# dropbox/divans

Measured on AMD Instinct MI355X. Metric: MB/s encode+decode per GPU, 64 KiB metablocks; bit-exact vs CPU, higher is better.
Workload: dtype u16/u64 integer

## Files before the change

### divans_amd/csrc/lit_bucket.hip

```cpp
#include "lit_bucket_dev.h"

namespace divans_hip {

__global__ __launch_bounds__(BK_SORT_THREADS) void bucket_sort_kernel(const BucketBatch b) {
    __shared__ __attribute__((aligned(16))) uint8_t staging[BK_PIECE];
    __shared__ __attribute__((aligned(16))) uint8_t piece_in[16 + BK_PIECE];
    __shared__ uint32_t hist[4][256];
    __shared__ uint32_t scan[256];
    const uint32_t s = blockIdx.x / b.pieces, piece = blockIdx.x % b.pieces;
    const uint32_t tid = threadIdx.x, w = tid >> 6, lane = tid & 63;
    const uint32_t len = b.in_sizes ? b.in_sizes[s] : b.stream_len;
    const uint8_t* in = b.in + (b.in_offsets ? b.in_offsets[s] : (uint64_t)s * b.stream_len);
    uint32_t* desc = b.desc + ((size_t)s * 256u + tid) * 8u + piece;
    const uint32_t base = piece * BK_PIECE;
    if (base >= len) { *desc = 0u; return; }
    const uint32_t n = len - base < BK_PIECE ? len - base : BK_PIECE;
    const size_t pl = b.slot;
    for (uint32_t i = tid; i < 1024u; i += BK_SORT_THREADS) (&hist[0][0])[i] = 0u;
    {
        const uint8_t* src = in + base;
        if ((((uintptr_t)src) & 15u) == 0u) {
            for (uint32_t i = tid * 16u; i < n; i += BK_SORT_THREADS * 16u) {
                if (i + 16u <= n) *(u32x4*)(piece_in + 16u + i) = *(const u32x4*)(src + i);
                else for (uint32_t k = i; k < n; ++k) piece_in[16u + k] = src[k];
            }
        } else {
            for (uint32_t i = tid; i < n; i += BK_SORT_THREADS) piece_in[16u + i] = src[i];
        }
        if (tid == 0u) piece_in[15] = base ? in[base - 1u] : 0u;
    }
    __syncthreads();
    const uint8_t* key_of = piece_in + 15;
    for (uint32_t bt = 0; bt < 32u; ++bt) {
        const uint32_t p = w * 2048u + bt * 64u + lane;
        if (p < n) atomicAdd(&hist[w][key_of[p]], 1u);
    }
    __syncthreads();
    const uint32_t c0 = hist[0][tid], c1 = hist[1][tid], c2 = hist[2][tid], c3 = hist[3][tid];
    const uint32_t tot = c0 + c1 + c2 + c3;
    scan[tid] = tot;
    __syncthreads();
    for (uint32_t d = 1; d < 256u; d <<= 1) {
        const uint32_t v = tid >= d ? scan[tid - d] : 0u;
        __syncthreads();
        scan[tid] += v;
        __syncthreads();
    }
    const uint32_t start = scan[tid] - tot;
    hist[0][tid] = start; hist[1][tid] = start + c0; hist[2][tid] = start + c0 + c1; hist[3][tid] = start + c0 + c1 + c2;
    *desc = start | (tot << 16);
    __syncthreads();
    uint16_t* inv = b.inv + (size_t)s * pl + base;
    for (uint32_t bt = 0; bt < 32u; ++bt) {
        const uint32_t p = w * 2048u + bt * 64u + lane;
        const bool valid = p < n;
        const uint32_t key = valid ? key_of[p] : 0u;
        const uint32_t byte = valid ? key_of[p + 1u] : 0u;
        unsigned long long same = __ballot(valid);
        for (uint32_t bit = 0; bit < 8u; ++bit) {
            const bool set = (key >> bit) & 1u;
            const unsigned long long bb = __ballot(set);
            same &= set ? bb : ~bb;
        }
        const uint32_t rank = lanes_below(same), cnt = (uint32_t)__popcll(same);
        if (valid) {
            const uint32_t off = hist[w][key];
            staging[off + rank] = (uint8_t)byte;
            inv[p] = (uint16_t)(off + rank);
            if (rank == cnt - 1u) hist[w][key] = off + cnt;
        }
    }
    __syncthreads();
    uint8_t* sorted = b.sorted + (size_t)s * pl + base;
    for (uint32_t i = tid * 16u; i < n; i += BK_SORT_THREADS * 16u) {
        if (i + 16u <= n) *(u32x4*)(sorted + i) = *(const u32x4*)(staging + i);
        else for (uint32_t k = i; k < n; ++k) sorted[k] = staging[k];
    }
}

__global__ __launch_bounds__(1024) void bucket_tasks_kernel(const BucketBatch b) {
    __shared__ uint32_t cnt[BK_CLASSES], basev[BK_CLASSES];
    const uint32_t t = blockIdx.x * 1024u + threadIdx.x;
    const uint32_t cap = b.n_streams * 256u;
    if (threadIdx.x < BK_CLASSES) cnt[threadIdx.x] = 0u;
    __syncthreads();
    uint32_t tot = 0;
    if (t < cap) {
        const u32x4* d = (const u32x4*)(b.desc + (size_t)t * 8u);
        const u32x4 d0 = d[0], d1 = d[1];
        tot = (d0.x >> 16) + (d0.y >> 16) + (d0.z >> 16) + (d0.w >> 16) + (d1.x >> 16) + (d1.y >> 16) + (d1.z >> 16) + (d1.w >> 16);
    }
    const int cls = bk_class_of(tot);
    uint32_t local = 0;
    for (int c = 0; c < (int)BK_CLASSES; ++c) {
        const unsigned long long m = __ballot(cls == c);
        if (m == 0ull) continue;
        const int leader = __ffsll((long long)m) - 1;
        uint32_t wbase = 0;
        if ((int)(threadIdx.x & 63u) == leader) wbase = atomicAdd(&cnt[c], (uint32_t)__popcll(m));
        wbase = (uint32_t)__builtin_amdgcn_readlane((int)wbase, leader);
        if (cls == c) local = wbase + lanes_below(m);
    }
    __syncthreads();
    if (threadIdx.x < BK_CLASSES) basev[threadIdx.x] = cnt[threadIdx.x] ? atomicAdd(&b.counters[threadIdx.x], cnt[threadIdx.x]) : 0u;
    __syncthreads();
    if (cls >= 0) b.tasks[(size_t)cls * cap + basev[cls] + local] = t;
}

__global__ __launch_bounds__(64) void bucket_chain_kernel(const BucketBatch b) {
    extern __shared__ __attribute__((aligned(16))) uint32_t lds32[];
    const uint32_t lane = threadIdx.x;
    uint32_t* my = lds32 + lane * BK_LANE_DWORDS;
    uint32_t* mydesc = my + BK_DESC_DW;
    uint32_t* tab = lds32 + BK_TAB_DW;
    const uint32_t inc = (uint32_t)b.inc; const int lim = b.lim;
    for (uint32_t i = lane; i < 128u; i += 64u) {
        const uint32_t sym = i >> 3, k = i & 7u;
        tab[i] = (2u * k >= sym ? inc : 0u) | (2u * k + 1u >= sym ? inc << 16 : 0u);
    }
    __syncthreads();
    const size_t pl = b.slot;
    const uint32_t cap = b.n_streams * 256u;
    BkTaskLists lists; lists.load(b.counters);
    const uint32_t total = lists.total();
    const u32x4 def0 = {4u | (8u << 16), 12u | (16u << 16), 20u | (24u << 16), 28u | (32u << 16)};
    const u32x4 def1 = {36u | (40u << 16), 44u | (48u << 16), 52u | (56u << 16), 60u | (64u << 16)};

    bool has_task = false, exhausted = false;
    uint32_t run_i = 0, nruns = 0, left = 0, idx = 0;
    u32x2* cur_sfs = b.sfs; const uint8_t* cur_sorted = b.sorted;
    uint32_t nt_stage = 0, nt_tid = 0;
    u32x4 nd0 = {0u, 0u, 0u, 0u}, nd1 = {0u, 0u, 0u, 0u};
    uint32_t win_cur = 0, win_end = 0, nxt_val = 0, nxt_w = 0;
    const uint32_t long_end = lists.ends[3];
    bool nxt_pending = false, drained = false;
    u32x2 e_next = {0u, 0u}; uint32_t m_next = 0;
    u32x2 pv0 = {0u, 0u}, pv1 = pv0, pv2 = pv0, pv3 = pv0, pv4 = pv0, pv5 = pv0, pv6 = pv0, pv7 = pv0;
    uint32_t m_prev = 0; u32x2* sfs_prev = b.sfs;

#define BK_OPAQUE(X) asm volatile("" : "+v"(X))
#define BK_BYTE(K, WORD, PV)                                                                            \
    if (((K - first) & 15u) < cnt) {                                                                    \
        const uint32_t byte_ = (WORD >> (8u * (K & 3u))) & 0xffu;                                       \
        const uint32_t hi = byte_ >> 4, lo = byte_ & 15u;                                               \
        uint32_t* rowl = my + 8u * (1u + hi);                                                           \
        BkRow H = bk_read(my, tab, hi), L = bk_read(rowl, tab, lo);                                     \
        const u32x2 v = {bk_pack(H, hi), bk_pack(L, lo)};                                               \
        H.w0 += H.a0; H.w1 += H.a1; L.w0 += L.a0; L.w1 += L.a1;           \
        if ((int)(H.w1.w >> 16) >= lim) bk_renorm(H);                                                   \
        if ((int)(L.w1.w >> 16) >= lim) bk_renorm(L);                                                   \
        *(u32x4*)my = H.w0; *(u32x4*)(my + 4) = H.w1; *(u32x4*)rowl = L.w0; *(u32x4*)(rowl + 4) = L.w1; \
        PV = v;                                                                                         \
    }

    for (;;) {
        u32x2 e = e_next; const uint32_t m = m_next;
        if (m_prev & BK_VALID) {
            u32x2* dst = sfs_prev + (m_prev & 0xffffu);
            const uint32_t pf = (m_prev >> 16) & 15u, pc = (m_prev >> 20) & 15u;
            if (pc == 8u) {
                const u32x4 q0 = {pv0.x, pv0.y, pv1.x, pv1.y}, q1 = {pv2.x, pv2.y, pv3.x, pv3.y};
                const u32x4 q2 = {pv4.x, pv4.y, pv5.x, pv5.y}, q3 = {pv6.x, pv6.y, pv7.x, pv7.y};
                bk_store_quad((u32x4*)dst, q0); bk_store_quad((u32x4*)(dst + 2), q1);
                bk_store_quad((u32x4*)(dst + 4), q2); bk_store_quad((u32x4*)(dst + 6), q3);
            } else {
                if (((0u - pf) & 15u) < pc) bk_store_pair(dst + 0, pv0);
                if (((1u - pf) & 15u) < pc) bk_store_pair(dst + 1, pv1);
                if (((2u - pf) & 15u) < pc) bk_store_pair(dst + 2, pv2);
                if (((3u - pf) & 15u) < pc) bk_store_pair(dst + 3, pv3);
                if (((4u - pf) & 15u) < pc) bk_store_pair(dst + 4, pv4);
                if (((5u - pf) & 15u) < pc) bk_store_pair(dst + 5, pv5);
                if (((6u - pf) & 15u) < pc) bk_store_pair(dst + 6, pv6);
                if (((7u - pf) & 15u) < pc) bk_store_pair(dst + 7, pv7);
            }
        }
        {
            const bool adv = has_task && left == 0u, more = run_i < nruns;
            const uint32_t d = mydesc[run_i & 7u];
            if (adv && more) { left = d >> 16; idx = d & 0xffffu; ++run_i; }
            if (adv && !more) has_task = false;
        }
        {
            const bool fetch_ = has_task && left != 0u;
            const uint32_t base = idx & ~7u, first_ = idx & 7u;
            const uint32_t cnt_ = left < 8u - first_ ? left : 8u - first_;
            const uint8_t* lp = fetch_ ? cur_sorted + base : b.sorted;
            e_next = *(const u32x2*)lp;
            m_next = fetch_ ? (base | (first_ << 16) | (cnt_ << 20) | BK_VALID) : 0u;
            idx += fetch_ ? cnt_ : 0u; left -= fetch_ ? cnt_ : 0u;
        }
        BK_OPAQUE(e);
        m_prev = m; sfs_prev = cur_sfs;
        if (m & BK_VALID) {
            const uint32_t first = (m >> 16) & 15u, cnt = (m >> 20) & 15u;
            BK_BYTE(0u, e.x, pv0) BK_BYTE(1u, e.x, pv1) BK_BYTE(2u, e.x, pv2) BK_BYTE(3u, e.x, pv3)
            BK_BYTE(4u, e.y, pv4) BK_BYTE(5u, e.y, pv5) BK_BYTE(6u, e.y, pv6) BK_BYTE(7u, e.y, pv7)
        }
        if (!has_task && !(m_next & BK_VALID) && nt_stage == 3u) {
            BK_OPAQUE(nd0); BK_OPAQUE(nd1);
            uint32_t n = 0;
            const uint32_t dsc[8] = {nd0.x, nd0.y, nd0.z, nd0.w, nd1.x, nd1.y, nd1.z, nd1.w};
#pragma unroll
            for (uint32_t j = 0; j < 8u; ++j) if (dsc[j] >> 16) { mydesc[n] = dsc[j] + j * BK_PIECE; ++n; }
            nruns = n; run_i = 0u;
            for (uint32_t r = 0; r < 17u; ++r) { *(u32x4*)(my + 8u * r) = def0; *(u32x4*)(my + 8u * r + 4u) = def1; }
            cur_sfs = b.sfs + (size_t)(nt_tid >> 8) * pl; cur_sorted = b.sorted + (size_t)(nt_tid >> 8) * pl;
            left = 0u; has_task = true; nt_stage = 0u;
        }
        const bool want = nt_stage == 0u && !exhausted;
        if (nt_stage == 2u) nt_stage = 3u;
        else if (nt_stage == 1u) {
            BK_OPAQUE(nt_tid);
            const u32x4* dp = (const u32x4*)(b.desc + (size_t)nt_tid * 8u);
            nd0 = dp[0]; nd1 = dp[1];
            nt_stage = 2u;
        }
        const unsigned long long wm = __ballot(want);
        if (wm) {
            if (win_cur == win_end && nxt_pending) {
                BK_OPAQUE(nxt_val);
                const uint32_t basev = (uint32_t)__builtin_amdgcn_readfirstlane((int)nxt_val);
                nxt_pending = false;
                if (basev >= total) { drained = true; win_cur = win_end = total; }
                else { win_cur = basev; win_end = basev + nxt_w < total ? basev + nxt_w : total; }
            }
            const uint32_t avail = win_end - win_cur, asked = (uint32_t)__popcll(wm);
            const uint32_t rank = lanes_below(wm);
            if (want) {
                if (rank < avail) {
                    const uint32_t t = win_cur + rank;
                    nt_tid = *lists.at(b.tasks, cap, t);
                    nt_stage = 1u;
                } else if (drained) exhausted = true;
            }
            win_cur += asked < avail ? asked : avail;
        }
        const uint32_t want_w = win_end < long_end ? 64u : BK_WINDOW;
        if (!nxt_pending && !drained && win_end - win_cur < want_w / 2u) {
            nxt_w = want_w;
            if (lane == 0u) nxt_val = atomicAdd(&b.counters[BK_CLAIM], want_w);
            nxt_pending = true;
        }
        const bool done = !has_task && !(m_next & BK_VALID) && !(m_prev & BK_VALID) && nt_stage == 0u && exhausted;
        if (__ballot(!done) == 0ull) break;
    }
#undef BK_BYTE
#undef BK_OPAQUE
}

__global__ __launch_bounds__(1024) void bucket_unsort_kernel(const BucketBatch b) {
    __shared__ u32x2 buf[BK_PIECE];
    const uint32_t s = blockIdx.x / b.pieces, piece = blockIdx.x % b.pieces;
    const uint32_t len = b.in_sizes ? b.in_sizes[s] : b.stream_len;
    const uint32_t base = piece * BK_PIECE;
    if (base >= len) return;
    const uint32_t n = len - base < BK_PIECE ? len - base : BK_PIECE;
    const size_t pl = b.slot;
    const u32x2* src = b.sfs + (size_t)s * pl + base;
    for (uint32_t i = threadIdx.x; i < n; i += 1024u) buf[i] = __builtin_nontemporal_load(src + i);
    __syncthreads();
    const uint16_t* inv = b.inv + (size_t)s * pl + base;
    u32x2* dst = (u32x2*)(b.sf + (size_t)s * b.sf_stride) + base;
    for (uint32_t i = threadIdx.x; i < n; i += 1024u) dst[i] = buf[inv[i]];
}

__global__ __launch_bounds__(1024) void bucket_unsort32_kernel(const BucketBatch b) {
    __shared__ uint32_t buf[BK_PIECE];
    const uint32_t s = blockIdx.x / b.pieces, piece = blockIdx.x % b.pieces;
    const uint32_t len = b.in_sizes ? b.in_sizes[s] : b.stream_len;
    const uint32_t base = piece * BK_PIECE;
    if (base >= len) return;
    const uint32_t n = len - base < BK_PIECE ? len - base : BK_PIECE;
    const size_t pl = b.slot;
    const uint32_t* src = (const uint32_t*)b.sfs + (size_t)s * pl + base;
    const uint32_t n2 = (n + 1u) & ~1u;
    for (uint32_t i = 2u * threadIdx.x; i < n2; i += 2048u) *(u32x2*)(buf + i) = __builtin_nontemporal_load((const u32x2*)(src + i));
    __syncthreads();
    const uint16_t* inv = b.inv + (size_t)s * pl + base;
    uint32_t* dst = b.sf + (size_t)s * b.sf_stride + base;
    for (uint32_t i = 2u * threadIdx.x; i < n2; i += 2048u) {
        const uint32_t iv = *(const uint32_t*)(inv + i);
        const u32x2 v = {buf[iv & 0xffffu], i + 1u < n ? buf[iv >> 16] : 0u};
        *(u32x2*)(dst + i) = v;
    }
}

uint32_t bucket_chain_lds_bytes() { return (64u * BK_LANE_DWORDS + 128u) * 4u; }

void launch_bucket_tasks(const BucketBatch& b, hipStream_t st) {
    hipLaunchKernelGGL(bucket_tasks_kernel, dim3((b.n_streams + 3u) / 4u), dim3(1024), 0, st, b);
}
void launch_bucket_unsort(const BucketBatch& b, hipStream_t st) {
    hipLaunchKernelGGL(bucket_unsort_kernel, dim3(b.n_streams * b.pieces), dim3(1024), 0, st, b);
}

void launch_bucket_unsort32(const BucketBatch& b, hipStream_t st) {
    hipLaunchKernelGGL(bucket_unsort32_kernel, dim3(b.n_streams * b.pieces), dim3(1024), 0, st, b);
}

hipError_t launch_bucket_model(const BucketBatch& b, uint32_t chain_blocks, hipStream_t st) {
    hipError_t e = hipMemsetAsync(b.counters, 0, 64, st);
    if (e != hipSuccess) return e;
    if (b.pieces < 8u) {
        e = hipMemsetAsync(b.desc, 0, (size_t)b.n_streams * 256u * 8u * sizeof(uint32_t), st);
        if (e != hipSuccess) return e;
    }
    hipLaunchKernelGGL(bucket_sort_kernel, dim3(b.n_streams * b.pieces), dim3(BK_SORT_THREADS), 0, st, b);
    hipLaunchKernelGGL(bucket_tasks_kernel, dim3((b.n_streams + 3u) / 4u), dim3(1024), 0, st, b);
    hipLaunchKernelGGL(bucket_chain_kernel, dim3(chain_blocks), dim3(64), bucket_chain_lds_bytes(), st, b);
    hipLaunchKernelGGL(bucket_unsort_kernel, dim3(b.n_streams * b.pieces), dim3(1024), 0, st, b);
    return hipGetLastError();
}

}
```

### divans_amd/csrc/lit_bucket_dev.h

```cpp
#ifndef DIVANS_LIT_BUCKET_DEV_H_
#define DIVANS_LIT_BUCKET_DEV_H_
#include "lit_device.h"

namespace divans_hip {

constexpr uint32_t BK_PIECE = 8192;
constexpr uint32_t BK_SORT_THREADS = 256;
constexpr uint32_t BK_LANE_DWORDS = 148;
constexpr uint32_t BK_DESC_DW = 136;
constexpr uint32_t BK_TAB_DW = 64 * BK_LANE_DWORDS;
constexpr uint32_t BK_VALID = 1u << 31;
constexpr uint32_t BK_WINDOW = 256;
constexpr uint32_t BK_CLASSES = 6;
constexpr uint32_t BK_CLAIM = 8;

__device__ __forceinline__ int bk_class_of(uint32_t tot) {
    return tot == 0u ? -1 : (tot >= 16384u ? 0 : (tot >= 8192u ? 1 : (tot >= 4096u ? 2 : (tot >= 2048u ? 3 : (tot >= 64u ? 4 : 5)))));
}
struct BkTaskLists {
    uint32_t ends[BK_CLASSES];
    __device__ __forceinline__ void load(const uint32_t* counters) {
        uint32_t acc = 0;
#pragma unroll
        for (uint32_t c = 0; c < BK_CLASSES; ++c) { acc += counters[c]; ends[c] = acc; }
    }
    __device__ __forceinline__ uint32_t total() const { return ends[BK_CLASSES - 1u]; }
    __device__ __forceinline__ const uint32_t* at(const uint32_t* tasks, uint32_t cap, uint32_t t) const {
        uint32_t cls = 0, base = 0;
#pragma unroll
        for (uint32_t c = 0; c + 1u < BK_CLASSES; ++c) if (t >= ends[c]) { cls = c + 1u; base = ends[c]; }
        return tasks + (size_t)cls * cap + (t - base);
    }
};

__device__ __forceinline__ uint32_t lanes_below(unsigned long long m) {
    return __builtin_amdgcn_mbcnt_hi((uint32_t)(m >> 32), __builtin_amdgcn_mbcnt_lo((uint32_t)m, 0u));
}

struct BkRow { u32x4 w0, w1, a0, a1; int chi, cprev; };

__device__ __forceinline__ BkRow bk_read(const uint32_t* row, const uint32_t* tab, uint32_t sym) {
    BkRow r;
    r.w0 = *(const u32x4*)row; r.w1 = *(const u32x4*)(row + 4);
    const uint16_t* r16 = (const uint16_t*)row;
    r.chi = r16[sym];
    r.cprev = r16[sym ? sym - 1u : 0u];
    r.a0 = *(const u32x4*)(tab + sym * 8u); r.a1 = *(const u32x4*)(tab + sym * 8u + 4u);
    return r;
}
__device__ __forceinline__ uint32_t bk_pack(const BkRow& r, uint32_t sym) {
    const int mx = (int)(r.w1.w >> 16);
    const int clo = sym ? r.cprev : 0;
    const float rcp = biased_rcp15(mx);
    const uint32_t dhi = scaled_div(r.chi, mx, rcp), dlo = scaled_div(clo, mx, rcp);
    return (dlo + 1u) | ((dhi - dlo - 1u) << 16);
}
__device__ __forceinline__ void bk_renorm(BkRow& r) {
    const u32x4 b0 = {1u | (2u << 16), 3u | (4u << 16), 5u | (6u << 16), 7u | (8u << 16)};
    const u32x4 b1 = {9u | (10u << 16), 11u | (12u << 16), 13u | (14u << 16), 15u | (16u << 16)};
    const u32x4 t0 = r.w0 + b0, t1 = r.w1 + b1;
    r.w0 = t0 - ((t0 >> 2) & 0x3fff3fffu);
    r.w1 = t1 - ((t1 >> 2) & 0x3fff3fffu);
}

__device__ __forceinline__ void bk_store_quad(u32x4* p, u32x4 v) {
    asm volatile("global_store_dwordx4 %0, %1, off" : : "v"(p), "v"(v) : "memory");
}
__device__ __forceinline__ void bk_store_pair(u32x2* p, u32x2 v) {
    asm volatile("global_store_dwordx2 %0, %1, off" : : "v"(p), "v"(v) : "memory");
}
__device__ __forceinline__ void bk_store_word(uint32_t* p, uint32_t v) {
    asm volatile("global_store_dword %0, %1, off" : : "v"(p), "v"(v) : "memory");
}

}
#endif
```

Measured before the change: 14680.

## Keep chain high row and run descriptors in registers, swizzle LDS rows, wave-scan sort

In the chain kernel, the high-nibble CDF row and the run descriptors now live in VGPRs instead of per-lane LDS. Descriptors are picked via a bitmask and register select, and the low rows use an XOR swizzle by lane to spread LDS banks. This shrinks per-lane LDS from 148 to 128 dwords and cuts LDS reads and writes per byte. The sort kernel replaces the block-wide LDS scan with a wave-shuffle scan plus per-wave totals, and replaces the 8-ballot key match with LDS atomic-or masks, which may be slower under heavy key collisions and costs more VGPR pressure.

```diff
diff --git a/divans_amd/csrc/lit_bucket.hip b/divans_amd/csrc/lit_bucket.hip
--- a/divans_amd/csrc/lit_bucket.hip
+++ b/divans_amd/csrc/lit_bucket.hip
@@ -6,7 +6,8 @@
     __shared__ __attribute__((aligned(16))) uint8_t staging[BK_PIECE];
     __shared__ __attribute__((aligned(16))) uint8_t piece_in[16 + BK_PIECE];
     __shared__ uint32_t hist[4][256];
-    __shared__ uint32_t scan[256];
+    __shared__ unsigned long long lane_masks[4][256];
+    __shared__ uint32_t wave_tot[4];
     const uint32_t s = blockIdx.x / b.pieces, piece = blockIdx.x % b.pieces;
     const uint32_t tid = threadIdx.x, w = tid >> 6, lane = tid & 63;
     const uint32_t len = b.in_sizes ? b.in_sizes[s] : b.stream_len;
@@ -16,7 +17,7 @@
     if (base >= len) { *desc = 0u; return; }
     const uint32_t n = len - base < BK_PIECE ? len - base : BK_PIECE;
     const size_t pl = b.slot;
-    for (uint32_t i = tid; i < 1024u; i += BK_SORT_THREADS) (&hist[0][0])[i] = 0u;
+    for (uint32_t i = tid; i < 1024u; i += BK_SORT_THREADS) { (&hist[0][0])[i] = 0u; (&lane_masks[0][0])[i] = 0ull; }
     {
         const uint8_t* src = in + base;
         if ((((uintptr_t)src) & 15u) == 0u) {
@@ -38,32 +39,29 @@
     __syncthreads();
     const uint32_t c0 = hist[0][tid], c1 = hist[1][tid], c2 = hist[2][tid], c3 = hist[3][tid];
     const uint32_t tot = c0 + c1 + c2 + c3;
-    scan[tid] = tot;
-    __syncthreads();
-    for (uint32_t d = 1; d < 256u; d <<= 1) {
-        const uint32_t v = tid >= d ? scan[tid - d] : 0u;
-        __syncthreads();
-        scan[tid] += v;
-        __syncthreads();
-    }
-    const uint32_t start = scan[tid] - tot;
+    uint32_t incl = tot;
+#pragma unroll
+    for (uint32_t d = 1; d < 64u; d <<= 1) {
+        const uint32_t v = (uint32_t)__shfl_up((int)incl, d, 64);
+        if (lane >= d) incl += v;
+    }
+    if (lane == 63u) wave_tot[w] = incl;
+    __syncthreads();
+    uint32_t start = incl - tot;
+    for (uint32_t k = 0; k < w; ++k) start += wave_tot[k];
     hist[0][tid] = start; hist[1][tid] = start + c0; hist[2][tid] = start + c0 + c1; hist[3][tid] = start + c0 + c1 + c2;
     *desc = start | (tot << 16);
     __syncthreads();
     uint16_t* inv = b.inv + (size_t)s * pl + base;
+    unsigned long long* masks = lane_masks[w];
     for (uint32_t bt = 0; bt < 32u; ++bt) {
         const uint32_t p = w * 2048u + bt * 64u + lane;
-        const bool valid = p < n;
-        const uint32_t key = valid ? key_of[p] : 0u;
-        const uint32_t byte = valid ? key_of[p + 1u] : 0u;
-        unsigned long long same = __ballot(valid);
-        for (uint32_t bit = 0; bit < 8u; ++bit) {
-            const bool set = (key >> bit) & 1u;
-            const unsigned long long bb = __ballot(set);
-            same &= set ? bb : ~bb;
-        }
-        const uint32_t rank = lanes_below(same), cnt = (uint32_t)__popcll(same);
-        if (valid) {
+        if (p < n) {
+            const uint32_t key = key_of[p], byte = key_of[p + 1u];
+            __hip_atomic_fetch_or(&masks[key], 1ull << lane, __ATOMIC_RELAXED, __HIP_MEMORY_SCOPE_WORKGROUP);
+            const unsigned long long same = __hip_atomic_load(&masks[key], __ATOMIC_RELAXED, __HIP_MEMORY_SCOPE_WORKGROUP);
+            __hip_atomic_store(&masks[key], 0ull, __ATOMIC_RELAXED, __HIP_MEMORY_SCOPE_WORKGROUP);
+            const uint32_t rank = lanes_below(same), cnt = (uint32_t)__popcll(same);
             const uint32_t off = hist[w][key];
             staging[off + rank] = (uint8_t)byte;
             inv[p] = (uint16_t)(off + rank);
@@ -109,9 +107,8 @@
 
 __global__ __launch_bounds__(64) void bucket_chain_kernel(const BucketBatch b) {
     extern __shared__ __attribute__((aligned(16))) uint32_t lds32[];
-    const uint32_t lane = threadIdx.x;
+    const uint32_t lane = threadIdx.x, sw = lane & 15u;
     uint32_t* my = lds32 + lane * BK_LANE_DWORDS;
-    uint32_t* mydesc = my + BK_DESC_DW;
     uint32_t* tab = lds32 + BK_TAB_DW;
     const uint32_t inc = (uint32_t)b.inc; const int lim = b.lim;
     for (uint32_t i = lane; i < 128u; i += 64u) {
@@ -119,6 +116,7 @@
         tab[i] = (2u * k >= sym ? inc : 0u) | (2u * k + 1u >= sym ? inc << 16 : 0u);
     }
     __syncthreads();
+#define BK_BUMP(W0, W1, SYM) { W0 += *(const u32x4*)(tab + (SYM) * 8u); W1 += *(const u32x4*)(tab + (SYM) * 8u + 4u); }
     const size_t pl = b.slot;
     const uint32_t cap = b.n_streams * 256u;
     BkTaskLists lists; lists.load(b.counters);
@@ -127,7 +125,8 @@
     const u32x4 def1 = {36u | (40u << 16), 44u | (48u << 16), 52u | (56u << 16), 60u | (64u << 16)};
 
     bool has_task = false, exhausted = false;
-    uint32_t run_i = 0, nruns = 0, left = 0, idx = 0;
+    uint32_t runs = 0, left = 0, idx = 0;
+    u32x4 cd0 = {0u, 0u, 0u, 0u}, cd1 = cd0, h0 = def0, h1 = def1;
     u32x2* cur_sfs = b.sfs; const uint8_t* cur_sorted = b.sorted;
     uint32_t nt_stage = 0, nt_tid = 0;
     u32x4 nd0 = {0u, 0u, 0u, 0u}, nd1 = {0u, 0u, 0u, 0u};
@@ -143,13 +142,14 @@
     if (((K - first) & 15u) < cnt) {                                                                    \
         const uint32_t byte_ = (WORD >> (8u * (K & 3u))) & 0xffu;                                       \
         const uint32_t hi = byte_ >> 4, lo = byte_ & 15u;                                               \
-        uint32_t* rowl = my + 8u * (1u + hi);                                                           \
-        BkRow H = bk_read(my, tab, hi), L = bk_read(rowl, tab, lo);                                     \
-        const u32x2 v = {bk_pack(H, hi), bk_pack(L, lo)};                                               \
-        H.w0 += H.a0; H.w1 += H.a1; L.w0 += L.a0; L.w1 += L.a1;           \
-        if ((int)(H.w1.w >> 16) >= lim) bk_renorm(H);                                                   \
-        if ((int)(L.w1.w >> 16) >= lim) bk_renorm(L);                                                   \
-        *(u32x4*)my = H.w0; *(u32x4*)(my + 4) = H.w1; *(u32x4*)rowl = L.w0; *(u32x4*)(rowl + 4) = L.w1; \
+        const uint32_t c0 = ((2u * hi) ^ sw) << 2;                                                      \
+        u32x4* rl0 = (u32x4*)(my + c0); u32x4* rl1 = (u32x4*)(my + (c0 ^ 4u));                          \
+        u32x4 l0 = *rl0, l1 = *rl1;                                                                     \
+        const u32x2 v = {bk_pack_row(h0, h1, hi), bk_pack_row(l0, l1, lo)};                             \
+        BK_BUMP(h0, h1, hi); BK_BUMP(l0, l1, lo);                                                       \
+        if ((int)(h1.w >> 16) >= lim) bk_renorm_row(h0, h1);                                            \
+        if ((int)(l1.w >> 16) >= lim) bk_renorm_row(l0, l1);                                            \
+        *rl0 = l0; *rl1 = l1;                                                                           \
         PV = v;                                                                                         \
     }
 
@@ -175,9 +175,11 @@
             }
         }
         {
-            const bool adv = has_task && left == 0u, more = run_i < nruns;
-            const uint32_t d = mydesc[run_i & 7u];
-            if (adv && more) { left = d >> 16; idx = d & 0xffffu; ++run_i; }
+            const bool adv = has_task && left == 0u, more = runs != 0u;
+            const uint32_t j = (uint32_t)__builtin_ctz(runs | 256u);
+            uint32_t d, d_unused_;
+            bk_pick2(cd0, cd1, j & 7u, d, d_unused_);
+            if (adv && more) { left = d >> 16; idx = (d & 0xffffu) + j * BK_PIECE; runs &= runs - 1u; }
             if (adv && !more) has_task = false;
         }
         {
@@ -198,12 +200,11 @@
         }
         if (!has_task && !(m_next & BK_VALID) && nt_stage == 3u) {
             BK_OPAQUE(nd0); BK_OPAQUE(nd1);
-            uint32_t n = 0;
-            const uint32_t dsc[8] = {nd0.x, nd0.y, nd0.z, nd0.w, nd1.x, nd1.y, nd1.z, nd1.w};
-#pragma unroll
-            for (uint32_t j = 0; j < 8u; ++j) if (dsc[j] >> 16) { mydesc[n] = dsc[j] + j * BK_PIECE; ++n; }
-            nruns = n; run_i = 0u;
-            for (uint32_t r = 0; r < 17u; ++r) { *(u32x4*)(my + 8u * r) = def0; *(u32x4*)(my + 8u * r + 4u) = def1; }
+            cd0 = nd0; cd1 = nd1;
+            runs = (nd0.x >> 16 ? 1u : 0u) | (nd0.y >> 16 ? 2u : 0u) | (nd0.z >> 16 ? 4u : 0u) | (nd0.w >> 16 ? 8u : 0u)
+                 | (nd1.x >> 16 ? 16u : 0u) | (nd1.y >> 16 ? 32u : 0u) | (nd1.z >> 16 ? 64u : 0u) | (nd1.w >> 16 ? 128u : 0u);
+            h0 = def0; h1 = def1;
+            for (uint32_t c = 0; c < 32u; ++c) *(u32x4*)(my + 4u * c) = ((c ^ sw) & 1u) ? def1 : def0;
             cur_sfs = b.sfs + (size_t)(nt_tid >> 8) * pl; cur_sorted = b.sorted + (size_t)(nt_tid >> 8) * pl;
             left = 0u; has_task = true; nt_stage = 0u;
         }
@@ -245,6 +246,7 @@
         if (__ballot(!done) == 0ull) break;
     }
 #undef BK_BYTE
+#undef BK_BUMP
 #undef BK_OPAQUE
 }
 
@@ -285,7 +287,7 @@
     }
 }
 
-uint32_t bucket_chain_lds_bytes() { return (64u * BK_LANE_DWORDS + 128u) * 4u; }
+uint32_t bucket_chain_lds_bytes() { return (BK_TAB_DW + 128u) * 4u; }
 
 void launch_bucket_tasks(const BucketBatch& b, hipStream_t st) {
     hipLaunchKernelGGL(bucket_tasks_kernel, dim3((b.n_streams + 3u) / 4u), dim3(1024), 0, st, b);
diff --git a/divans_amd/csrc/lit_bucket_dev.h b/divans_amd/csrc/lit_bucket_dev.h
--- a/divans_amd/csrc/lit_bucket_dev.h
+++ b/divans_amd/csrc/lit_bucket_dev.h
@@ -6,8 +6,7 @@
 
 constexpr uint32_t BK_PIECE = 8192;
 constexpr uint32_t BK_SORT_THREADS = 256;
-constexpr uint32_t BK_LANE_DWORDS = 148;
-constexpr uint32_t BK_DESC_DW = 136;
+constexpr uint32_t BK_LANE_DWORDS = 128;
 constexpr uint32_t BK_TAB_DW = 64 * BK_LANE_DWORDS;
 constexpr uint32_t BK_VALID = 1u << 31;
 constexpr uint32_t BK_WINDOW = 256;
@@ -55,14 +54,32 @@
     const uint32_t dhi = scaled_div(r.chi, mx, rcp), dlo = scaled_div(clo, mx, rcp);
     return (dlo + 1u) | ((dhi - dlo - 1u) << 16);
 }
-__device__ __forceinline__ void bk_renorm(BkRow& r) {
+__device__ __forceinline__ void bk_renorm_row(u32x4& w0, u32x4& w1) {
     const u32x4 b0 = {1u | (2u << 16), 3u | (4u << 16), 5u | (6u << 16), 7u | (8u << 16)};
     const u32x4 b1 = {9u | (10u << 16), 11u | (12u << 16), 13u | (14u << 16), 15u | (16u << 16)};
-    const u32x4 t0 = r.w0 + b0, t1 = r.w1 + b1;
-    r.w0 = t0 - ((t0 >> 2) & 0x3fff3fffu);
-    r.w1 = t1 - ((t1 >> 2) & 0x3fff3fffu);
+    const u32x4 t0 = w0 + b0, t1 = w1 + b1;
+    w0 = t0 - ((t0 >> 2) & 0x3fff3fffu);
+    w1 = t1 - ((t1 >> 2) & 0x3fff3fffu);
 }
+__device__ __forceinline__ void bk_renorm(BkRow& r) { bk_renorm_row(r.w0, r.w1); }
 
+__device__ __forceinline__ void bk_pick2(const u32x4& w0, const u32x4& w1, uint32_t k, uint32_t& cur, uint32_t& prv) {
+    const bool b2 = (k & 4u) != 0u, b1 = (k & 2u) != 0u, b0 = (k & 1u) != 0u;
+    const uint32_t x = b2 ? w1.x : w0.x, y = b2 ? w1.y : w0.y, z = b2 ? w1.z : w0.z, w = b2 ? w1.w : w0.w;
+    const uint32_t px = b2 ? w0.w : 0u, py = x, pz = y, pw = z;
+    cur = b0 ? (b1 ? w : y) : (b1 ? z : x);
+    prv = b0 ? (b1 ? pw : py) : (b1 ? pz : px);
+}
+__device__ __forceinline__ uint32_t bk_pack_row(const u32x4& w0, const u32x4& w1, uint32_t sym) {
+    uint32_t cur, prv;
+    bk_pick2(w0, w1, sym >> 1, cur, prv);
+    const uint32_t pair = (sym & 1u) ? cur : __builtin_amdgcn_alignbit(cur, prv, 16);
+    const int mx = (int)(w1.w >> 16);
+    const int chi = (int)(pair >> 16), clo = (int)(pair & 0xffffu);
+    const float rcp = biased_rcp15(mx);
+    const uint32_t dhi = scaled_div(chi, mx, rcp), dlo = scaled_div(clo, mx, rcp);
+    return (dlo + 1u) | ((dhi - dlo - 1u) << 16);
+}
 __device__ __forceinline__ void bk_store_quad(u32x4* p, u32x4 v) {
     asm volatile("global_store_dwordx4 %0, %1, off" : : "v"(p), "v"(v) : "memory");
 }
```

Measured after the change: 14710 (median of 6 runs). No clear change (+0.3%).

## Software-pipeline LDS reads across byte slots in bucket chain kernel

Applied to the files above, without the earlier changes.

Restructures the per-byte CDF update loop so the high-nibble row lives in registers and the next byte's LDS reads are issued before the current byte's division and pack, hiding LDS latency. Inactive slots now run predicated, using a zero-increment table row and an infinite limit instead of branching. The body is gated on a wave ballot. Renormalization uses packed 16-bit ops, and row initialization moves before the first barrier. The trade-off is higher register pressure, wasted work on inactive slots, and reliance on asm fences for ordering.

```diff
diff --git a/divans_amd/csrc/lit_bucket.hip b/divans_amd/csrc/lit_bucket.hip
--- a/divans_amd/csrc/lit_bucket.hip
+++ b/divans_amd/csrc/lit_bucket.hip
@@ -107,6 +107,23 @@
     if (cls >= 0) b.tasks[(size_t)cls * cap + basev[cls] + local] = t;
 }
 
+struct BkSlot { u32x4 lw0, lw1, la0, la1, ha0, ha1; int hchi, hcprev, lchi, lcprev, lim; uint32_t hi, lo; uint32_t* rowl; };
+
+__device__ __forceinline__ BkSlot bk_slot_read(uint32_t* my, const uint32_t* tab, uint32_t byte, bool active, int lim) {
+    BkSlot s;
+    s.hi = byte >> 4; s.lo = byte & 15u;
+    s.rowl = my + 8u * (1u + s.hi);
+    const uint16_t* h16 = (const uint16_t*)my; const uint16_t* l16 = (const uint16_t*)s.rowl;
+    s.hchi = h16[s.hi]; s.hcprev = h16[s.hi ? s.hi - 1u : 0u];
+    s.lw0 = *(const u32x4*)s.rowl; s.lw1 = *(const u32x4*)(s.rowl + 4);
+    s.lchi = l16[s.lo]; s.lcprev = l16[s.lo ? s.lo - 1u : 0u];
+    s.lim = active ? lim : 0x7fffffff;
+    const uint32_t* th = tab + (active ? s.hi : 16u) * 8u; const uint32_t* tl = tab + (active ? s.lo : 16u) * 8u;
+    s.ha0 = *(const u32x4*)th; s.ha1 = *(const u32x4*)(th + 4);
+    s.la0 = *(const u32x4*)tl; s.la1 = *(const u32x4*)(tl + 4);
+    return s;
+}
+
 __global__ __launch_bounds__(64) void bucket_chain_kernel(const BucketBatch b) {
     extern __shared__ __attribute__((aligned(16))) uint32_t lds32[];
     const uint32_t lane = threadIdx.x;
@@ -114,17 +131,19 @@
     uint32_t* mydesc = my + BK_DESC_DW;
     uint32_t* tab = lds32 + BK_TAB_DW;
     const uint32_t inc = (uint32_t)b.inc; const int lim = b.lim;
-    for (uint32_t i = lane; i < 128u; i += 64u) {
+    for (uint32_t i = lane; i < BK_CHAIN_TAB_DW; i += 64u) {
         const uint32_t sym = i >> 3, k = i & 7u;
         tab[i] = (2u * k >= sym ? inc : 0u) | (2u * k + 1u >= sym ? inc << 16 : 0u);
     }
-    __syncthreads();
     const size_t pl = b.slot;
     const uint32_t cap = b.n_streams * 256u;
     BkTaskLists lists; lists.load(b.counters);
     const uint32_t total = lists.total();
     const u32x4 def0 = {4u | (8u << 16), 12u | (16u << 16), 20u | (24u << 16), 28u | (32u << 16)};
     const u32x4 def1 = {36u | (40u << 16), 44u | (48u << 16), 52u | (56u << 16), 60u | (64u << 16)};
+    for (uint32_t r = 0; r < 17u; ++r) { *(u32x4*)(my + 8u * r) = def0; *(u32x4*)(my + 8u * r + 4u) = def1; }
+    __syncthreads();
+    u32x4 hw0 = def0, hw1 = def1;
 
     bool has_task = false, exhausted = false;
     uint32_t run_i = 0, nruns = 0, left = 0, idx = 0;
@@ -139,18 +158,23 @@
     uint32_t m_prev = 0; u32x2* sfs_prev = b.sfs;
 
 #define BK_OPAQUE(X) asm volatile("" : "+v"(X))
-#define BK_BYTE(K, WORD, PV)                                                                            \
-    if (((K - first) & 15u) < cnt) {                                                                    \
-        const uint32_t byte_ = (WORD >> (8u * (K & 3u))) & 0xffu;                                       \
-        const uint32_t hi = byte_ >> 4, lo = byte_ & 15u;                                               \
-        uint32_t* rowl = my + 8u * (1u + hi);                                                           \
-        BkRow H = bk_read(my, tab, hi), L = bk_read(rowl, tab, lo);                                     \
-        const u32x2 v = {bk_pack(H, hi), bk_pack(L, lo)};                                               \
-        H.w0 += H.a0; H.w1 += H.a1; L.w0 += L.a0; L.w1 += L.a1;           \
-        if ((int)(H.w1.w >> 16) >= lim) bk_renorm(H);                                                   \
-        if ((int)(L.w1.w >> 16) >= lim) bk_renorm(L);                                                   \
-        *(u32x4*)my = H.w0; *(u32x4*)(my + 4) = H.w1; *(u32x4*)rowl = L.w0; *(u32x4*)(rowl + 4) = L.w1; \
-        PV = v;                                                                                         \
+#define BK_FENCE(A, B, C, D, E, F) asm volatile("" : "+v"(A), "+v"(B), "+v"(C), "+v"(D), "+v"(E), "+v"(F) : : "memory")
+#define BK_ARRIVE(PV, T)                                                                                                          \
+    asm volatile("" : "+v"(PV.x), "+v"(PV.y), "+v"(T.lw0), "+v"(T.lw1), "+v"(T.la0), "+v"(T.la1), "+v"(T.ha0), "+v"(T.ha1),       \
+                      "+v"(T.hchi), "+v"(T.hcprev), "+v"(T.lchi), "+v"(T.lcprev) : : "memory")
+#define BK_SLOT(K, PV, NEXT_WORD)                                                                                              \
+    {                                                                                                                          \
+        int hmx = (int)(hw1.w >> 16), lmx = (int)(S.lw1.w >> 16);                                                              \
+        int hchi = S.hchi, hcprev = S.hcprev, lchi = S.lchi, lcprev = S.lcprev;                                                \
+        const uint32_t hi = S.hi, lo = S.lo;                                                                                   \
+        hw0 += S.ha0; hw1 += S.ha1; S.lw0 += S.la0; S.lw1 += S.la1;                              \
+        if ((int)(hw1.w >> 16) >= S.lim) bk_renorm_pk(hw0, hw1);                                                               \
+        if ((int)(S.lw1.w >> 16) >= S.lim) bk_renorm_pk(S.lw0, S.lw1);                                                         \
+        *(u32x4*)my = hw0; *(u32x4*)(my + 4) = hw1; *(u32x4*)S.rowl = S.lw0; *(u32x4*)(S.rowl + 4) = S.lw1;                    \
+        if (K < 7u) S = bk_slot_read(my, tab, ((NEXT_WORD) >> (8u * ((K + 1u) & 3u))) & 0xffu, ((K + 1u - first) & 15u) < cnt, lim); \
+        BK_FENCE(hmx, lmx, hchi, hcprev, lchi, lcprev);                                                                        \
+        PV.x = bk_pack3(hchi, hcprev, hmx, hi); PV.y = bk_pack3(lchi, lcprev, lmx, lo);                                        \
+        if (K < 7u) BK_ARRIVE(PV, S);                                                                                          \
     }
 
     for (;;) {
@@ -191,10 +215,11 @@
         }
         BK_OPAQUE(e);
         m_prev = m; sfs_prev = cur_sfs;
-        if (m & BK_VALID) {
+        if (__ballot((m & BK_VALID) != 0u)) {
             const uint32_t first = (m >> 16) & 15u, cnt = (m >> 20) & 15u;
-            BK_BYTE(0u, e.x, pv0) BK_BYTE(1u, e.x, pv1) BK_BYTE(2u, e.x, pv2) BK_BYTE(3u, e.x, pv3)
-            BK_BYTE(4u, e.y, pv4) BK_BYTE(5u, e.y, pv5) BK_BYTE(6u, e.y, pv6) BK_BYTE(7u, e.y, pv7)
+            BkSlot S = bk_slot_read(my, tab, e.x & 0xffu, ((0u - first) & 15u) < cnt, lim);
+            BK_SLOT(0u, pv0, e.x) BK_SLOT(1u, pv1, e.x) BK_SLOT(2u, pv2, e.x) BK_SLOT(3u, pv3, e.y)
+            BK_SLOT(4u, pv4, e.y) BK_SLOT(5u, pv5, e.y) BK_SLOT(6u, pv6, e.y) BK_SLOT(7u, pv7, e.y)
         }
         if (!has_task && !(m_next & BK_VALID) && nt_stage == 3u) {
             BK_OPAQUE(nd0); BK_OPAQUE(nd1);
@@ -204,6 +229,7 @@
             for (uint32_t j = 0; j < 8u; ++j) if (dsc[j] >> 16) { mydesc[n] = dsc[j] + j * BK_PIECE; ++n; }
             nruns = n; run_i = 0u;
             for (uint32_t r = 0; r < 17u; ++r) { *(u32x4*)(my + 8u * r) = def0; *(u32x4*)(my + 8u * r + 4u) = def1; }
+            hw0 = def0; hw1 = def1;
             cur_sfs = b.sfs + (size_t)(nt_tid >> 8) * pl; cur_sorted = b.sorted + (size_t)(nt_tid >> 8) * pl;
             left = 0u; has_task = true; nt_stage = 0u;
         }
@@ -244,7 +270,9 @@
         const bool done = !has_task && !(m_next & BK_VALID) && !(m_prev & BK_VALID) && nt_stage == 0u && exhausted;
         if (__ballot(!done) == 0ull) break;
     }
-#undef BK_BYTE
+#undef BK_SLOT
+#undef BK_FENCE
+#undef BK_ARRIVE
 #undef BK_OPAQUE
 }
 
@@ -285,7 +313,7 @@
     }
 }
 
-uint32_t bucket_chain_lds_bytes() { return (64u * BK_LANE_DWORDS + 128u) * 4u; }
+uint32_t bucket_chain_lds_bytes() { return (64u * BK_LANE_DWORDS + BK_CHAIN_TAB_DW) * 4u; }
 
 void launch_bucket_tasks(const BucketBatch& b, hipStream_t st) {
     hipLaunchKernelGGL(bucket_tasks_kernel, dim3((b.n_streams + 3u) / 4u), dim3(1024), 0, st, b);
diff --git a/divans_amd/csrc/lit_bucket_dev.h b/divans_amd/csrc/lit_bucket_dev.h
--- a/divans_amd/csrc/lit_bucket_dev.h
+++ b/divans_amd/csrc/lit_bucket_dev.h
@@ -9,6 +9,7 @@
 constexpr uint32_t BK_LANE_DWORDS = 148;
 constexpr uint32_t BK_DESC_DW = 136;
 constexpr uint32_t BK_TAB_DW = 64 * BK_LANE_DWORDS;
+constexpr uint32_t BK_CHAIN_TAB_DW = 17 * 8;
 constexpr uint32_t BK_VALID = 1u << 31;
 constexpr uint32_t BK_WINDOW = 256;
 constexpr uint32_t BK_CLASSES = 6;
@@ -63,6 +64,25 @@
     r.w1 = t1 - ((t1 >> 2) & 0x3fff3fffu);
 }
 
+typedef uint16_t bk_u16x2 __attribute__((ext_vector_type(2)));
+__device__ __forceinline__ uint32_t bk_renorm_dword(uint32_t w, uint32_t bias) {
+    const bk_u16x2 t = __builtin_bit_cast(bk_u16x2, w) + __builtin_bit_cast(bk_u16x2, bias);
+    const bk_u16x2 two = {2, 2};
+    return __builtin_bit_cast(uint32_t, (bk_u16x2)(t - (t >> two)));
+}
+__device__ __forceinline__ void bk_renorm_pk(u32x4& w0, u32x4& w1) {
+    w0.x = bk_renorm_dword(w0.x, 1u | (2u << 16)); w0.y = bk_renorm_dword(w0.y, 3u | (4u << 16));
+    w0.z = bk_renorm_dword(w0.z, 5u | (6u << 16)); w0.w = bk_renorm_dword(w0.w, 7u | (8u << 16));
+    w1.x = bk_renorm_dword(w1.x, 9u | (10u << 16)); w1.y = bk_renorm_dword(w1.y, 11u | (12u << 16));
+    w1.z = bk_renorm_dword(w1.z, 13u | (14u << 16)); w1.w = bk_renorm_dword(w1.w, 15u | (16u << 16));
+}
+__device__ __forceinline__ uint32_t bk_pack3(int chi, int cprev, int mx, uint32_t sym) {
+    const int clo = sym ? cprev : 0;
+    const float rcp = biased_rcp15(mx);
+    const uint32_t dhi = scaled_div(chi, mx, rcp), dlo = scaled_div(clo, mx, rcp);
+    return (dlo + 1u) | ((dhi - dlo - 1u) << 16);
+}
+
 __device__ __forceinline__ void bk_store_quad(u32x4* p, u32x4 v) {
     asm volatile("global_store_dwordx4 %0, %1, off" : : "v"(p), "v"(v) : "memory");
 }
```

Measured after the change: 14980 before, 15110 after (median of 6 runs). No clear change (+0.9%).
